# Jiraiya812/Fast-CU-Decision-HEVC

Hardware: AMD Instinct MI355X
Metric: CTUs/sec (RDO decision only) at 4K all-intra (higher is better)
Workload: dtype int32+f64

## Files before the change

fast-cu-decision-hevc_amd/csrc/fcu_engine.h:

```cpp
#pragma once
#include <stdint.h>
#include <string.h>
#include <type_traits>
#include "../../include/fcu.h"

#ifdef FCU_EMU
#include <math.h>
#include <stdio.h>
#include <stdlib.h>
#define FCU_DEV static inline
#define FCU_MEMBER inline
#define FCU_NOINLINE
#define FCU_INLINE
#define FCU_TABLE static const
static int g_emu_phase = 0, g_emu_in_phase = 0, g_emu_lane = 0, g_emu_relax = 0;
#define FCU_EMU_RELAX(on) (g_emu_relax = (on))
static inline int fcu_emu_phase_begin() { g_emu_phase++; g_emu_in_phase = 1; g_emu_lane = 0; return 0; }
static inline int fcu_emu_phase_next(int lane) { if (lane + 1 >= 64) g_emu_in_phase = 0; g_emu_lane = lane + 1; return lane + 1; }
template <class T> static inline T fcu_emu_uni(T v, int site, int line)
{
  enum { SITES = 2048, K = 32, B = 16 };
  struct Seen { int phase, first, cur, idx, n; unsigned char vals[K][B]; };
  static Seen seen[SITES];
  if (g_emu_in_phase && !g_emu_relax && sizeof(T) <= B && site < SITES) {
// ... 106 lines not shown
#define FCU_TIC(v) do { } while (0)
#define FCU_TOC(E_, v, idx) do { } while (0)
#define FCU_COUNT(E_, idx, n) do { } while (0)
#endif
#ifndef FCU_QTOC
#define FCU_QTIC(v) do { } while (0)
#define FCU_QTOC(E_, v, idx) do { } while (0)
#endif
#ifndef FCU_ITOC
#define FCU_ITOC(E_, v, idx) do { } while (0)
#endif
#ifndef FCU_MTOC
#define FCU_MTOC(E_, v, idx) do { } while (0)
#endif
#ifndef FCU_STOC
#define FCU_STOC(E_, v, idx) do { } while (0)
#define FCU_SPATH(E_, path) do { } while (0)
#define FCU_S7_COEFF(E_, v, comp) do { } while (0)
#endif

#include "fcu_tables.h"

struct HotTables { uint32_t bin[256]; uint16_t scan[3][16]; uint8_t scan_cg8[3][4]; uint8_t ctx_ind_map4x4[16]; uint8_t group_idx[32];
                   uint64_t scan4_nib[3], map4_nib; uint32_t cnt_bits[4]; };
#ifdef FCU_EMU
static HotTables g_hot;
#else
__shared__ HotTables g_hot;
#endif

#if defined(FCU_PROFILE_RQT) && !defined(FCU_EMU)
#define FCU_RTIC(v) long long v = clock64()
#define FCU_RTOC(P_, v, idx) do { if (!SER && threadIdx.x == 0) { ((Chain *)((char *)&(P_) - __builtin_offsetof(Chain, p)))->prof[idx] += (unsigned long long)(clock64() - v); v = clock64(); } } while (0)
#elif defined(FCU_PROFILE_RDOQ) && !defined(FCU_EMU)
#define FCU_RTIC(v) long long v = clock64()
#define FCU_RTOC(P_, v, idx) do { if ((FCU_PROFILE_RDOQ + 0) == 2 ? (!SER && threadIdx.x == 0) : SER) { ((Chain *)((char *)&(P_) - __builtin_offsetof(Chain, p)))->prof[idx] += (unsigned long long)(clock64() - v); v = clock64(); } } while (0)
#else
#define FCU_RTIC(v) do { } while (0)
#define FCU_RTOC(P_, v, idx) do { } while (0)
#endif
namespace fcu {

enum { CTU = 64, MAXDEPTH = 3, NPART = 256, LOG2_MAXTU = 5, LOG2_MINTU = 2, TU_MAXDEPTH_INTRA = 3 };
enum { SIZE_2Nx2N = 0, SIZE_2NxN = 1, SIZE_Nx2N = 2, SIZE_NxN = 3, SIZE_2NxnU = 4, SIZE_2NxnD = 5, SIZE_nLx2N = 6, SIZE_nRx2N = 7, SIZE_NONE = 8, MODE_INTER = 0, MODE_INTRA = 1, MODE_NONE = 2 };
enum { SLICE_I = 0, SLICE_P = 1 };
enum { PLANAR = 0, DC = 1, HOR = 10, VER = 26, DM_CHROMA = 36 };
enum { CTX_SPLIT = 0, CTX_PARTSIZE = 3, CTX_INTRA_LUMA = 4, CTX_CHROMA_PRED = 5, CTX_CBF_LUMA = 6, CTX_CBF_CHROMA = 11,
// ... 87 lines not shown
  Cabac c64_state[5][4]; uint32_t c64_distk[5][4];
  Yuv16 resi_cu, resi_best, qt_resi[4];
  Yuv tmp_pred;
  uint8_t me_pred[9][CTU * CTU];
  int16_t me_h[3][72 * 64];
  int par_ps[4];
  int memo_valid[4][MEMO_K], memo_next[4], memo_zero[4][MEMO_K];
  int16_t memo_mv[4][MEMO_K][NPART][2]; int8_t memo_ref[4][MEMO_K][NPART];
  uint8_t memo_tr_idx[4][MEMO_K][NPART], memo_cbf[4][MEMO_K][3][NPART], memo_tskip[4][MEMO_K][3][NPART];
  alignas(16) int16_t memo_coef[MEMO_K * MEMO_POOL], memo_resi[MEMO_K * MEMO_POOL];
};

struct Env { Chain *C; Scratch *G; int cur_ctu, slice_start; int16_t tx0, ty0, tx1, ty1; };
FCU_DEV int in_tile(const Env E, int cx, int cy) { return cx >= E.tx0 && cx < E.tx1 && cy >= E.ty0 && cy < E.ty1; }
struct TU { int log2, tr_depth, part, nparts, x, y, off_y, cw, cwo, cx, cy, c_tr_depth, c_code_all, off_c, cu_depth, plast; };

struct Shared {
  Cabac cab[1 + (MAXDEPTH + 1) + MAXLC + 1];
  uint8_t ref5[5][68]; int dc5[5]; uint32_t cm_dist[5];
  union {
    int16_t lane_abs[MAXLC][32];
    RdoqRec rq_rec[16];
    int32_t rq_grp[16][MAXVC];
    struct {
      int32_t colsum[128];
      union {
        struct { uint8_t ref[264], reff[264]; };
        uint8_t ref5b[5][68];
      };
    };
  };
  union {
    int16_t rq_lv[16];
    uint32_t sad[36];
  };
  int dc;
  int ref_tag;
  int best_idx[4], reco_best_idx[4];
  union {
    struct { int rd_mode[12]; int n_rd; int preds[3]; int n_mpm; };
    int uni[8];
  };
  union {
    struct {
      uint8_t vc_slot[MAXVC];
      int vc_abs[MAXVC], vc_lsp[MAXVC], vc_last[MAXVC]; uint32_t vc_dist[MAXVC]; uint32_t vc_bits[MAXVC]; double vc_cost[MAXVC];
// ... 158 lines not shown
  int offset;
  if (log2 == 2) offset = g_hot.ctx_ind_map4x4[4 * py + px];
  else {
    int cnt; const int xs = px & 3, ys = py & 3;
    if (pattern == 0) { int t = xs + ys; cnt = (t >= 3) ? 0 : ((t >= 1) ? 1 : 2); }
    else if (pattern == 1) cnt = (ys >= 2) ? 0 : ((ys >= 1) ? 1 : 2);
    else if (pattern == 2) cnt = (xs >= 2) ? 0 : ((xs >= 1) ? 1 : 2);
    else cnt = 2;
    offset = ((((px >> 2) + (py >> 2)) > 0) ? (ch ? 0 : 3) : 0) + cnt;
  }
  return first + offset;
}
FCU_DEV int coef_remain_bins(uint32_t symbol, uint32_t rparam)
{
  int code = (int)symbol;
  if (code < (3 << rparam)) return (int)(((uint32_t)code >> rparam) + 1) + (int)rparam;
  uint32_t length = rparam;
  code -= 3 << rparam;
  while (code >= (1 << length)) code -= 1 << (length++);
  return (int)(3 + length + 1 - rparam) + (int)length;
}
#ifdef FCU_EMU
enum { WALK_RDOQ_CALLS, WALK_RDOQ_TOP_IS_GROUP0, WALK_RDOQ_AHEAD_GROUPS, WALK_RDOQ_ONLY_GROUP0, WALK_RDOQ_ONLY_LAST_GROUP, WALK_RDOQ_ALL_ZERO,
       WALK_BITS_CALLS, WALK_BITS_ONE_EMPTY_RUN_BETWEEN, WALK_BITS_SECOND_ROUND, WALK_N };
extern "C" { __attribute__((weak)) unsigned long long fcu_emu_walk_cnt[WALK_N]; }
static const int32_t *g_emu_lscan_lo = nullptr, *g_emu_lscan_hi = nullptr;
#define FCU_WALK_COUNT(i, n) (fcu_emu_walk_cnt[i] += (unsigned long long)(n))
#define FCU_CHECK_LSCAN(p) FCU_CHECK((const int32_t *)(p) >= g_emu_lscan_lo && (const int32_t *)(p) < g_emu_lscan_hi)
#else
#define FCU_WALK_COUNT(i, n) do { } while (0)
#define FCU_CHECK_LSCAN(p) do { } while (0)
#endif
template <int SER>
FCU_DEV FCU_INLINE void code_coeff_body(int c, const int16_t *coef, int st, int last, int log2, int comp, int scanType, int tsFlag, const Params &P_, int16_t *absCoeff)
{
  if (SER) { c = FCU_UNI(c); coef = FCU_UNI(coef); last = FCU_UNI(last); scanType = FCU_UNI(scanType); tsFlag = FCU_UNI(tsFlag); absCoeff = FCU_UNI(absCoeff); }
  const Params &P = *FCU_UNI(&P_);
  st = FCU_UNI(st); log2 = FCU_UNI(log2); comp = FCU_UNI(comp);
  FCU_IN_LDS(absCoeff);
  const FCU_HBM int16_t *coefg = (const FCU_HBM int16_t *)coef;
  const int ch = comp ? 1 : 0, N = 1 << log2; int n2 = N * N;
  if (last < 0 && st == 1 && n2 >= 64) {
    int q = (n2 >> 6) - 1;
    for (; q >= 0; q--) {
      uint32_t w[32];
      __builtin_memcpy(w, __builtin_assume_aligned((const void *)(coef + q * 64), 16), 128);
      uint32_t any = 0;
#pragma unroll
      for (int k = 0; k < 32; k++) any |= w[k];
      if (any) break;
    }
    if (q < 0) return;
    n2 = (q + 1) * 64;
  }
// ... 209 lines not shown
          for (int n = (lastCG == 1 ? last : 15); n >= 0; --n) {
            if (lv[n] != 0) {
              if (du[n] > 0) { curCost = -du[n]; curChange = 1; }
              else if (n == first && iabs(lv[n]) == 1) curCost = 0x7fffffff;
              else { curCost = du[n]; curChange = -1; }
            } else if (n < first) {
              const unsigned thisSign = srcg[(sub + n) * st] >= 0 ? 0 : 1;
              if (thisSign != signbit) curCost = 0x7fffffff; else { curCost = -du[n]; curChange = 1; }
            } else { curCost = -du[n]; curChange = 1; }
            if (curCost < minCostInc) { minCostInc = curCost; finalChange = curChange; minPos = n; }
          }
          if (lv[minPos] == 32767 || lv[minPos] == -32768) finalChange = -1;
          const int nv = srcg[(sub + minPos) * st] >= 0 ? lv[minPos] + finalChange : lv[minPos] - finalChange;
          dstg[(sub + minPos) * st] = (int16_t)nv;
        }
      }
      if (lastCG == 1) lastCG = 0;
    }
  }
  for (int sp = cgTop * 16 + 15; sp >= 0; sp--) if (dstg[sp * st]) { o.last = sp; break; }
  return o;
}

template <class CB>
FCU_DEV FCU_INLINE int rdoq_last_pos(CB cb, const FCU_HBM int16_t *dstg, const FCU_HBM RdoqRec *recg, const FCU_HBM double *cgg,
                                     int st, int log2, int ch, int scanType, int cbfCtx, const uint16_t *scan, const uint8_t *scanCG,
                                     uint64_t cgflag, int cgLastScanPos, int lastScanPos, double baseCost, double blockUncodedCost, double lambda)
{
  const int N = 1 << log2;
  double bestCost; int bestLastIdxP1 = 0;
  bestCost = blockUncodedCost + lambda * (double)cb(cbfCtx, 0);
  baseCost += lambda * (double)cb(cbfCtx, 1);
  const int lcc = log2 - 2, loff = ch ? 0 : (lcc * 3 + ((lcc + 1) >> 2)), lsh = ch ? lcc : ((lcc + 3) >> 2);
  const int lbx = CTX_LASTX + (ch ? 15 : 0) + loff, lby = CTX_LASTY + (ch ? 15 : 0) + loff, lgmax = g_hot.group_idx[N - 1];
  int foundLast = 0;
  for (int cgScanPos = cgLastScanPos; cgScanPos >= 0; cgScanPos--) {
    const int cgBlk = scanCG[cgScanPos];
    baseCost -= cgg[cgScanPos * st];
    if ((cgflag >> cgBlk) & 1) {
      const int top = (cgScanPos * 16 + 15 > lastScanPos) ? lastScanPos - cgScanPos * 16 : 15;
      int aLv = dstg[(cgScanPos * 16 + top) * st]; double aCs = recg[(cgScanPos * 16 + top) * st].cs;
      for (int posInCG = top; posInCG >= 0; posInCG--) {
        const int scanPos = cgScanPos * 16 + posInCG;
        const int lv = aLv; const double curCs = aCs;
        if (posInCG > 0) { aLv = dstg[(scanPos - 1) * st]; aCs = recg[(scanPos - 1) * st].cs; }
        if (lv) {
          const int blk = scan[scanPos];
          const int py = blk >> log2, px = blk - (py << log2);
          const int ax = scanType == 2 ? py : px, ay = scanType == 2 ? px : py;
          const int gx = g_hot.group_idx[ax], gy = g_hot.group_idx[ay];
          int bxs = 0, bys = 0;
          for (int k = 0; k < gx; k++) bxs += cb(lbx + (k >> lsh), 1);
          if (gx < lgmax) bxs += cb(lbx + (gx >> lsh), 0);
          for (int k = 0; k < gy; k++) bys += cb(lby + (k >> lsh), 1);
          if (gy < lgmax) bys += cb(lby + (gy >> lsh), 0);
          double r = (double)(bxs + bys);
          if (gx > 3) r += 32768.0 * (double)((gx - 2) >> 1);
          if (gy > 3) r += 32768.0 * (double)((gy - 2) >> 1);
          const double costLast = lambda * r;
          const double totalCost = baseCost + costLast - curCs;
          if (totalCost < bestCost) { bestLastIdxP1 = scanPos + 1; bestCost = totalCost; }
          if (lv > 1) { foundLast = 1; break; }
          baseCost -= recg[scanPos * st].cc; baseCost += recg[scanPos * st].c0;
        } else baseCost -= curCs;
      }
      if (foundLast) break;
    }
  }
  return bestLastIdxP1;
}
FCU_DEV FCU_INLINE int rdoq_signs(const FCU_HBM int32_t *srcg, FCU_HBM int16_t *dstg, int st, int bestLastIdxP1, int lastScanPos)
{
  int absSum = 0;
  for (int sp0 = 0; sp0 < bestLastIdxP1; sp0 += 16) {
    int lv[16]; int32_t sv[16];
#pragma unroll
    for (int k = 0; k < 16; k++) { const int ok = sp0 + k < bestLastIdxP1; lv[k] = ok ? dstg[(sp0 + k) * st] : 0; sv[k] = ok ? srcg[(sp0 + k) * st] : 0; }
#pragma unroll
    for (int k = 0; k < 16; k++) if (sp0 + k < bestLastIdxP1) { absSum += lv[k]; dstg[(sp0 + k) * st] = (int16_t)((sv[k] < 0) ? -lv[k] : lv[k]); }
  }
  for (int sp = bestLastIdxP1; sp <= lastScanPos; sp++) dstg[sp * st] = 0;

  return absSum;
}
FCU_DEV FCU_INLINE void rdoq_sign_hiding(const Params &P, const FCU_HBM int32_t *srcg, FCU_HBM int16_t *dstg, const FCU_HBM RdoqRec *recg, int st, int ch, int bestLastIdxP1, int absSum)
{
  if (P.sign_hiding && absSum >= 2) {
    const long long rdFactor = P.rd_factor[ch];
    int lastCG = -1;
    for (int subSet = (bestLastIdxP1 - 1) >> 4; subSet >= 0; subSet--) {
      const int subPos = subSet << 4; int firstNZ = 16, lastNZ = -1, sum = 0, n;
      uint32_t nzMask = 0, negMask = 0;
      {
        int lv16[16];
#pragma unroll
        for (int k = 0; k < 16; k++) lv16[k] = dstg[(subPos + k) * st];
#pragma unroll
        for (int k = 0; k < 16; k++) { sum += lv16[k]; nzMask |= (uint32_t)(lv16[k] != 0) << k; negMask |= (uint32_t)(lv16[k] < 0) << k; }
      }
      if (nzMask) { lastNZ = 31 - __builtin_clz(nzMask); firstNZ = __builtin_ctz(nzMask); }
      if (lastNZ >= 0 && lastCG == -1) lastCG = 1;
      if (lastNZ - firstNZ >= 4) {
        const uint32_t signbit = (negMask >> firstNZ) & 1;
        if (signbit != (uint32_t)(sum & 1)) {
          long long minCostInc = 0x7fffffffffffffffLL, curCost = 0x7fffffffffffffffLL;
          int minPos = -1, finalChange = 0, curChange = 0;
          for (n = (lastCG == 1 ? lastNZ : 15); n >= 0; --n) {
            const int sp = n + subPos; const int lv = dstg[sp * st]; const RdoqRec q = recg[sp * st];
            if (lv != 0) {
              const long long costUp = rdFactor * (-q.du) + q.up;
              long long costDown = rdFactor * (q.du) + q.dn - ((iabs(lv) == 1) ? q.sd : 0);
              if (lastCG == 1 && lastNZ == n && iabs(lv) == 1) costDown -= (4 << 15);
              if (costUp < costDown) { curCost = costUp; curChange = 1; }
              else { curChange = -1; if (n == firstNZ && iabs(lv) == 1) curCost = 0x7fffffffffffffffLL; else curCost = costDown; }
            } else {
              curCost = rdFactor * (-(long long)(iabs(q.du))) + (1 << 15) + q.up + q.sd;
              curChange = 1;
              if (n < firstNZ) { const uint32_t thissign = srcg[sp * st] >= 0 ? 0 : 1; if (thissign != signbit) curCost = 0x7fffffffffffffffLL; }
            }
            if (curCost < minCostInc) { minCostInc = curCost; finalChange = curChange; minPos = sp; }
          }
          const int old = dstg[minPos * st];
          if (old == 32767 || old == -32768) finalChange = -1;
          const int nv = srcg[minPos * st] >= 0 ? old + finalChange : old - finalChange;
          dstg[minPos * st] = (int16_t)nv;
        }
      }
      if (lastCG == 1) lastCG = 0;
    }
  }
}
template <int SER, class CB>
FCU_DEV FCU_INLINE RdoqOut rdoq_finish(CB cb, const Params &P, const FCU_HBM int32_t *srcg, FCU_HBM int16_t *dstg, FCU_HBM RdoqRec *recg, FCU_HBM double *cgg,
                                       int st, int log2, int ch, int scanType, int cbfCtx, const uint16_t *scan, const uint8_t *scanCG,
                                       uint64_t cgflag, int cgLastScanPos, int lastScanPos, double baseCost, double blockUncodedCost, double lambda)
{
  FCU_RTIC(rt_);
  const int bestLastIdxP1 = rdoq_last_pos(cb, dstg, recg, cgg, st, log2, ch, scanType, cbfCtx, scan, scanCG, cgflag, cgLastScanPos, lastScanPos, baseCost, blockUncodedCost, lambda);
  FCU_RTOC(P, rt_, 13);
  const int absSum = rdoq_signs(srcg, dstg, st, bestLastIdxP1, lastScanPos);
  FCU_RTOC(P, rt_, 14);
  rdoq_sign_hiding(P, srcg, dstg, recg, st, ch, bestLastIdxP1, absSum);
  FCU_RTOC(P, rt_, 15);
  int last = bestLastIdxP1 - 1;
  while (last >= 0 && dstg[last * st] == 0) last--;
  RdoqOut o = { absSum, last };
  return o;
}


template <int SER, int EST>
FCU_DEV FCU_NOINLINE RdoqOut rdoq(int c, const int32_t *src, int16_t *dst, int st, int topNZ, int log2, int comp, int scanType, int cbfCtx, const Params &P_, RdoqRec *rec, double *costCGSig, int slot = 0)
{
  const Params &P = *FCU_UNI(&P_);
  st = FCU_UNI(st); log2 = FCU_UNI(log2); comp = FCU_UNI(comp); cbfCtx = FCU_UNI(cbfCtx);
  if (SER) { c = FCU_UNI(c); src = FCU_UNI(src); dst = FCU_UNI(dst); topNZ = FCU_UNI(topNZ); scanType = FCU_UNI(scanType); rec = FCU_UNI(rec); costCGSig = FCU_UNI(costCGSig); }
  FCU_RTIC(rt_);
  if (topNZ < 0) { FCU_WALK_COUNT(WALK_RDOQ_ALL_ZERO, !SER); RdoqOut z = { 0, -1 }; return z; }
  const FCU_HBM int32_t *srcg = (const FCU_HBM int32_t *)src; FCU_HBM int16_t *dstg = (FCU_HBM int16_t *)dst;
  FCU_HBM RdoqRec *recg = (FCU_HBM RdoqRec *)rec; FCU_HBM double *cgg = (FCU_HBM double *)costCGSig;
  auto cb = [&](int ctx, int bin) -> int { return EST ? (int)FCU_EST[ctx * 2 + bin] : ctx_bits(c, ctx, bin); };
  const int ch = comp ? 1 : 0, N = 1 << log2, n2 = N * N;
  const int qp = comp ? P.qp_c : P.qp;
  const int qbits = rdoq_qbits(log2, qp);
  const double lambda = P.rdoq_lambda[comp];
  const double errScale = P.err_scale[ch][log2 - 2];
  const uint16_t *scan = log2 == 2 ? &g_hot.scan[scanType][0] : k_scan + k_scan_off[scanType * 4 + log2 - 2];
  const uint8_t *scanCG = log2 <= 3 ? g_hot.scan_cg8[log2 == 2 ? 0 : scanType] : k_scan_cg + k_scan_cg_off[scanType * 4 + log2 - 2];
  const int wg = N >> 2, firstSig = first_sig_ctx(log2, scanType, ch);
  const int sigOff = CTX_SIG + (ch ? 28 : 0), cgBase = CTX_SIGCG + (ch ? 2 : 0);
  uint64_t cgflag = 0;
  int cgLastScanPos = -1; uint32_t ctxSet = 0; int c1 = 1, c2 = 0;
  double baseCost = 0, blockUncodedCost = 0;
  int lastScanPos = -1; uint32_t c1Idx = 0, c2Idx = 0, goRice = 0;
  int absSum = 0;

  const uint64_t scan4 = g_hot.scan4_nib[scanType], map4 = g_hot.map4_nib;
  int g10 = 0, g10Ctx = -1;
  const int cgTop = topNZ >> 4;
  for (int cg = (n2 >> 4) - 1; cg > cgTop; cg--) {
    int32_t v[16];
#pragma unroll
    for (int k = 0; k < 16; k++) v[k] = srcg[(cg * 16 + k) * st];
#pragma unroll
    for (int k = 15; k >= 0; k--) { const double err = (double)iabs(v[k]); blockUncodedCost += err * err * errScale; }
  }
  baseCost = blockUncodedCost;
  FCU_RTOC(P, rt_, 11);
  constexpr bool GRP = !SER;
  int32_t ahead = 0, nxt[16];
  if (GRP) {
// ... 101 lines not shown
        rdCodedLevelandDist += cc - cs;
        rdUncodedDist += c0;
        if (posInCG != 0) nnzBeforePos0++;
      }
    }
    if (lastScanPos >= 0 && cgScanPos > 0) {
      ctxSet = (uint32_t)((ch ? 4 : 0) + ((!ch && (cgScanPos - 1) > 0) ? 2 : 0) + (c1 == 0));
      c1 = 1; c2 = 0; c1Idx = 0; c2Idx = 0; goRice = 0;
    }
    if (cgLastScanPos >= 0) {
      if (cgScanPos) {
        if (((cgflag >> cgBlk) & 1) == 0) {
          const int ctxSig = cgBase + sig_cg_ctx(cgflag, cgx, cgy, wg);
          baseCost += lambda * (double)cb(ctxSig, 0) - rdSigCost;
          cgg[cgScanPos * st] = lambda * (double)cb(ctxSig, 0);
        } else if (cgScanPos < cgLastScanPos) {
          if (nnzBeforePos0 == 0) { baseCost -= rdSigCost0; rdSigCost -= rdSigCost0; }
          double costZeroCG = baseCost;
          const int ctxSig = cgBase + sig_cg_ctx(cgflag, cgx, cgy, wg);
          baseCost += lambda * (double)cb(ctxSig, 1);
          costZeroCG += lambda * (double)cb(ctxSig, 0);
          cgg[cgScanPos * st] = lambda * (double)cb(ctxSig, 1);
          costZeroCG += rdUncodedDist; costZeroCG -= rdCodedLevelandDist; costZeroCG -= rdSigCost;
          if (costZeroCG < baseCost) {
            cgflag &= ~(1ull << cgBlk); baseCost = costZeroCG;
            cgg[cgScanPos * st] = lambda * (double)cb(ctxSig, 0);
            for (int posInCG = 15; posInCG >= 0; posInCG--) {
              const int scanPos = cgScanPos * 16 + posInCG;
              if (SER) { if (g_S.rq_lv[posInCG]) { g_S.rq_lv[posInCG] = 0; g_S.rq_rec[posInCG].cc = g_S.rq_rec[posInCG].c0; g_S.rq_rec[posInCG].cs = 0; } }
              else if (dstg[scanPos * st]) { dstg[scanPos * st] = 0; recg[scanPos * st].cc = recg[scanPos * st].c0; recg[scanPos * st].cs = 0; }
            }
          }
        }
      } else cgflag |= 1ull << cgBlk;
    }
    if (SER) {
#pragma unroll
      for (int k = 0; k < 16; k++) { recg[(cgScanPos * 16 + k) * st] = g_S.rq_rec[k]; dstg[(cgScanPos * 16 + k) * st] = g_S.rq_lv[k]; }
    }
  }
  FCU_RTOC(P, rt_, 12);
  if (lastScanPos < 0) { RdoqOut z = { 0, -1 }; return z; }
#ifdef FCU_EMU
  FCU_WALK_COUNT(WALK_RDOQ_ONLY_GROUP0, GRP && lastScanPos < 16);
  if (GRP && n2 > 16 && lastScanPos >= n2 - 16) {
    int other = 0;
    for (int sp = 0; sp < n2 - 16; sp++) other |= dstg[sp * st];
    FCU_WALK_COUNT(WALK_RDOQ_ONLY_LAST_GROUP, !other);
  }
#endif
  return rdoq_finish<SER>(cb, P, srcg, dstg, recg, cgg, st, log2, ch, scanType, cbfCtx, scan, scanCG, cgflag, cgLastScanPos, lastScanPos, baseCost, blockUncodedCost, lambda);
}

#ifdef FCU_EMU
template <class T> struct LaneVar {
  T v[64];
  LaneVar() { for (int i = 0; i < 64; i++) v[i] = T(); }
  void set(int lane, T x) { v[lane] = x; }
  T own(int lane) const { return v[lane]; }
  T get(int k) const { return v[k]; }
  void put(int k, T x) { v[k] = x; }
};
FCU_DEV uint32_t lane_mask16(const LaneVar<int> &f) { uint32_t m = 0; for (int k = 0; k < 16; k++) m |= (uint32_t)(f.v[k] != 0) << k; return m; }
#else
#if defined(__HIP_DEVICE_COMPILE__)
#define FCU_READLANE(v, k) __builtin_amdgcn_readlane((v), (k))
#define FCU_WRITELANE(val_, k_, old_) (((int)threadIdx.x == (k_)) ? (val_) : (old_))
#define FCU_BALLOT(p) __builtin_amdgcn_ballot_w64(p)
#else
#define FCU_READLANE(v, k) (v)
#define FCU_WRITELANE(val_, k_, old_) (val_)
#define FCU_BALLOT(p) ((unsigned long long)(p))
#endif
template <class T> struct LaneVar;
// ... 14 lines not shown
  { union { double d; int i[2]; } u, w; u.d = r; w.d = x; u.i[0] = FCU_WRITELANE(w.i[0], k, u.i[0]); u.i[1] = FCU_WRITELANE(w.i[1], k, u.i[1]); r = u.d; }
};
__device__ inline uint32_t lane_mask16(const LaneVar<int> &f) { return (uint32_t)FCU_BALLOT(f.r != 0) & 0xffffu; }
#endif

#ifndef FCU_WAVE_RDOQ_MIN_LOG2
#define FCU_WAVE_RDOQ_MIN_LOG2 2
#endif
FCU_DEV FCU_NOINLINE void rdoq_wave(int c, const int32_t *src, int16_t *dst, int topNZ, int log2, int comp, int scanType, int cbfCtx, const Params &P_, RdoqRec *rec, double *costCGSig)
{
  const Params &P = *FCU_UNI(&P_);
  c = FCU_UNI(c); src = FCU_UNI(src); dst = FCU_UNI(dst); topNZ = FCU_UNI(topNZ); log2 = FCU_UNI(log2); comp = FCU_UNI(comp);
  scanType = FCU_UNI(scanType); cbfCtx = FCU_UNI(cbfCtx); rec = FCU_UNI(rec); costCGSig = FCU_UNI(costCGSig);
  if (topNZ < 0) { FCU_SERIAL { g_S.rw_abs = 0; g_S.rw_lsp = -1; } return; }
  const FCU_HBM int32_t *srcg = (const FCU_HBM int32_t *)src; FCU_HBM int16_t *dstg = (FCU_HBM int16_t *)dst;
  FCU_HBM RdoqRec *recg = (FCU_HBM RdoqRec *)rec; FCU_HBM double *cgg = (FCU_HBM double *)costCGSig;
  auto cb = [&](int ctx, int bin) -> int { return (int)FCU_EST[ctx * 2 + bin]; };
  const int ch = comp ? 1 : 0, N = 1 << log2, n2 = N * N;
  const int qp = comp ? P.qp_c : P.qp;
  const int qbits = rdoq_qbits(log2, qp);
  const double lambda = P.rdoq_lambda[comp];
  const double errScale = P.err_scale[ch][log2 - 2];
  const uint16_t *scan = log2 == 2 ? &g_hot.scan[scanType][0] : k_scan + k_scan_off[scanType * 4 + log2 - 2];
  const uint8_t *scanCG = log2 <= 3 ? g_hot.scan_cg8[log2 == 2 ? 0 : scanType] : k_scan_cg + k_scan_cg_off[scanType * 4 + log2 - 2];
  const int wg = N >> 2, firstSig = first_sig_ctx(log2, scanType, ch);
  const int sigOff = CTX_SIG + (ch ? 28 : 0), cgBase = CTX_SIGCG + (ch ? 2 : 0);
  const uint64_t scan4 = g_hot.scan4_nib[scanType], map4 = g_hot.map4_nib;
  const int cgTop = topNZ >> 4;
  uint64_t cgflag = 0;
  int cgLastScanPos = -1; uint32_t ctxSet = 0; int c1 = 1, c2 = 0;
  double baseCost = 0, blockUncodedCost = 0;
  int lastScanPos = -1; uint32_t c1Idx = 0, c2Idx = 0, goRice = 0;
  int g10 = 0, g10Ctx = -1;
  for (int cg = (n2 >> 4) - 1; cg > cgTop; cg -= 4) {
    LaneVar<double> t0;
    FCU_FOR_LANES { const int g = cg - (lane >> 4); if (g > cgTop) { const double err = (double)iabs(srcg[g * 16 + (lane & 15)]); t0.set(lane, err * err * errScale); } }
    for (int j = 0; j < 4 && cg - j > cgTop; j++)
      for (int k = 15; k >= 0; k--) blockUncodedCost += t0.get(j * 16 + k);
  }
  baseCost = blockUncodedCost;
  LaneVar<int> vCgBlk, vNext;
  LaneVar<double> vCgSig;
  FCU_FOR_LANES { if (lane <= cgTop) vCgBlk.set(lane, scanCG[lane]); if (lane < 16) vNext.set(lane, srcg[cgTop * 16 + lane]); }
  for (int cgScanPos = cgTop; cgScanPos >= 0; cgScanPos--) {
    const int cgBlk = vCgBlk.get(cgScanPos), cgy = cgBlk / wg, cgx = cgBlk - cgy * wg;
    const int sigBase = sigOff + firstSig + ((!ch && (cgx + cgy) > 0) ? 3 : 0);
    const uint32_t cntBits = g_hot.cnt_bits[pattern_sig_ctx(cgflag, cgx, cgy, wg)];
// ... 171 lines not shown
      }
      for (int posInCG = top; posInCG >= 0; posInCG--) {
        const int lv = wLv.get(posInCG); const double curCs = wCs.get(posInCG);
        if (lv) {
          const double totalCost = baseCost + wCl.get(posInCG) - curCs;
          if (totalCost < bestCost) { bestLastIdxP1 = cgScanPos * 16 + posInCG + 1; bestCost = totalCost; }
          if (lv > 1) { foundLast = 1; break; }
          baseCost -= wCc.get(posInCG); baseCost += wC0.get(posInCG);
        } else baseCost -= curCs;
      }
    }
  }
  FCU_SERIAL { g_S.rw_abs = 0; }
  FCU_FOR_LANES {
    uint32_t acc = 0;
    for (int sp = lane; sp <= lastScanPos; sp += 64) {
      if (sp < bestLastIdxP1) { const int lv = dstg[sp]; acc += (uint32_t)lv; dstg[sp] = (int16_t)((srcg[sp] < 0) ? -lv : lv); }
      else dstg[sp] = 0;
    }
    FCU_WAVE_ADD((uint32_t *)&g_S.rw_abs, acc);
  }
  FCU_SERIAL {
    const int absSum = g_S.rw_abs;
    rdoq_sign_hiding(P, srcg, dstg, recg, 1, ch, bestLastIdxP1, absSum);
    int last = bestLastIdxP1 - 1;
    while (last >= 0 && dstg[last] == 0) last--;
    g_S.rw_lsp = last;
  }
}

FCU_DEV int use_filtered_ref(int mode, int log2, int isLuma)
{
  if (!isLuma || mode == DC) return 0;
  const int d1 = iabs(mode - HOR), d2 = iabs(mode - VER);
  return (d1 < d2 ? d1 : d2) > k_filter_thr[log2 - 2];
}
FCU_DEV int pred_pixel(const uint8_t *ref, int log2, int mode, int isLuma, int dc, int x, int y)
{
  const int N = 1 << log2;
  const uint8_t *corner = ref + 2 * N;
  if (mode == PLANAR)
    return ((N - 1 - x) * corner[-1 - y] + (x + 1) * corner[1 + N] + (N - 1 - y) * corner[1 + x] + (y + 1) * corner[-1 - N] + N) >> (log2 + 1);
  if (mode == DC) {
    int v = dc;
    if (isLuma && N <= 16) {
      if (x == 0 && y == 0) v = (corner[1] + corner[-1] + 2 * dc + 2) >> 2;
      else if (y == 0) v = (corner[1 + x] + 3 * dc + 2) >> 2;
      else if (x == 0) v = (corner[-1 - y] + 3 * dc + 2) >> 2;
    }
// ... 1869 lines not shown
      if (!((depth < ctu->depth[part] && depth < MAXDEPTH) || boundary)) {
        encode_cu_syntax(E, c, ctu, part, depth);
        const int rx = cx + s, ry = cy + s;
        if (((rx % CTU) == 0 || rx == P.width) && ((ry % CTU) == 0 || ry == P.height) && !lastCtuOfSlice) cab_trm(c, 0);
        sp--; continue;
      }
      stChild[sp] = 0;
    }
    if (stChild[sp] >= 4) { sp--; continue; }
    {
      const int qn = (NPART >> (2 * depth)) >> 2, p = part + stChild[sp] * qn;
      stChild[sp]++;
      if (ctu->x + part_x(p) < P.width && ctu->y + part_y(p) < P.height) { sp++; stPart[sp] = p; stChild[sp] = -1; }
    }
  }
}

FCU_DEV void load_hot_tables()
{
  FCU_FOR_LANES {
    for (int i = lane; i < 256; i += 64) g_hot.bin[i] = k_bin[i];
    for (int i = lane; i < 3 * 16; i += 64) { const int t = i / 16, j = i % 16; g_hot.scan[t][j] = k_scan[k_scan_off[t * 4 + 0] + j]; }
    if (lane < 12) g_hot.scan_cg8[lane / 4][lane % 4] = k_scan_cg[k_scan_cg_off[(lane / 4) * 4 + 1] + lane % 4];
    if (lane < 16) g_hot.ctx_ind_map4x4[lane] = k_ctx_ind_map4x4[lane];
    if (lane < 32) g_hot.group_idx[lane] = k_group_idx[lane];
    if (lane < 3) { uint64_t v = 0; for (int j = 0; j < 16; j++) v |= (uint64_t)k_scan[k_scan_off[lane * 4 + 0] + j] << (4 * j); g_hot.scan4_nib[lane] = v; }
    if (lane == 3) { uint64_t v = 0; for (int j = 0; j < 16; j++) v |= (uint64_t)k_ctx_ind_map4x4[j] << (4 * j); g_hot.map4_nib = v; }
    if (lane >= 4 && lane < 8) {
      const int pattern = lane - 4; uint32_t v = 0;
      for (int j = 0; j < 16; j++) {
        const int xs = j & 3, ys = j >> 2; int cnt;
        if (pattern == 0) { const int t = xs + ys; cnt = (t >= 3) ? 0 : ((t >= 1) ? 1 : 2); }
        else if (pattern == 1) cnt = (ys >= 2) ? 0 : ((ys >= 1) ? 1 : 2);
        else if (pattern == 2) cnt = (xs >= 2) ? 0 : ((xs >= 1) ? 1 : 2);
        else cnt = 2;
        v |= (uint32_t)cnt << (2 * j);
      }
      g_hot.cnt_bits[pattern] = v;
    }
  }
}

template <bool WPP = false>
FCU_DEV FCU_NOINLINE void compress_ctu(Chain *C, Scratch *G, int pos)
{
  C = FCU_UNI(C); G = FCU_UNI(G); pos = FCU_UNI(pos);
  Env E; E.C = C; E.G = G;
#ifdef FCU_EMU
  g_emu_lscan_lo = G->p_lscan; g_emu_lscan_hi = G->p_lscan + POOL;
#endif
  FCU_TIC(t10_);
  const Params &P = C->p;
  const int tileW = FCU_UNI(C->tile_w), tileX0 = FCU_UNI(C->tile_x0), tileY0 = FCU_UNI(C->tile_y0);
  const int col = pos % tileW;
  const int ctuRsAddr = FCU_UNI((tileY0 + pos / tileW) * C->w_ctu + tileX0 + col);
  E.tx0 = (int16_t)tileX0; E.ty0 = (int16_t)tileY0; E.tx1 = (int16_t)(tileX0 + tileW); E.ty1 = (int16_t)(tileY0 + FCU_UNI(C->tile_h));
  const int sliceLen = P.slice_ctus > 0 ? P.slice_ctus : C->n_ctu;
  const int sliceStart = (ctuRsAddr / sliceLen) * sliceLen;
  int sliceEnd = sliceStart + sliceLen; if (sliceEnd > C->n_ctu) sliceEnd = C->n_ctu;
  E.cur_ctu = ctuRsAddr; E.slice_start = sliceStart;
  fcu_ctu_out *out = &C->out[ctuRsAddr];
  const int x = (ctuRsAddr % C->w_ctu) * CTU, y = (ctuRsAddr / C->w_ctu) * CTU;
  const bool unit_start = ctuRsAddr == sliceStart || pos == 0;
  const bool row_start = WPP && col == 0 && !unit_start;
  FCU_SERIAL { g_S.env = E; g_S.ref_tag = -1; if (unit_start || row_start) cab_init(slot_ptr(E, 0, CI_CURR_BEST), P.qp, P.slice_type, P.cabac_b_table); else cab_copy1(slot_ptr(E, 0, CI_CURR_BEST), &C->state); }
  if (row_start && tileW >= 2) {
    const uint8_t *src = C->wpp_sync_in;
    FCU_FOR_LANES { Cabac *d = slot_ptr(E, 0, CI_CURR_BEST); for (int i = lane; i < NCTX; i += 64) d->ctx[i] = src[i]; }
  }
  FCU_FOR_LANES {
    for (int i = lane; i < NPART; i += 64) {
      out->depth[i] = 0; out->width[i] = CTU; out->height[i] = CTU; out->skip[i] = 0; out->part_size[i] = SIZE_NONE; out->pred_mode[i] = MODE_NONE;
// ... 112 lines not shown
```

Baseline: 20210.

## Prefetch RDOQ tail data in half-groups and cache scan tables in LDS

The last-position search in RDOQ now walks the coefficients in blocks of eight. It loads each block's levels and cost records ahead of use and stages the cs values in shared memory per slot, so global loads overlap with the serial cost evaluation. Sign hiding now batch-loads its record fields per half-group and returns the last nonzero position, which removes the separate backward scan; a mask-based helper covers the case without sign hiding. The 16x16 and 32x32 CG scan tables are copied into the shared hot-table struct. The cost is extra shared memory and more registers, plus emulator-only bounds checks and counters.

```diff
diff --git a/fast-cu-decision-hevc_amd/csrc/fcu_engine.h b/fast-cu-decision-hevc_amd/csrc/fcu_engine.h
--- a/fast-cu-decision-hevc_amd/csrc/fcu_engine.h
+++ b/fast-cu-decision-hevc_amd/csrc/fcu_engine.h
@@ -152,7 +152,8 @@
 #include "fcu_tables.h"
 
 struct HotTables { uint32_t bin[256]; uint16_t scan[3][16]; uint8_t scan_cg8[3][4]; uint8_t ctx_ind_map4x4[16]; uint8_t group_idx[32];
-                   uint64_t scan4_nib[3], map4_nib; uint32_t cnt_bits[4]; };
+                   uint64_t scan4_nib[3], map4_nib; uint32_t cnt_bits[4];
+                   uint8_t scan_cg16[16], scan_cg32[64]; };
 #ifdef FCU_EMU
 static HotTables g_hot;
 #else
@@ -286,6 +287,7 @@
     int16_t lane_abs[MAXLC][32];
     RdoqRec rq_rec[16];
     int32_t rq_grp[16][MAXVC];
+    double rq_cs[8][MAXVC];
     struct {
       int32_t colsum[128];
       union {
@@ -490,14 +492,24 @@
 }
 #ifdef FCU_EMU
 enum { WALK_RDOQ_CALLS, WALK_RDOQ_TOP_IS_GROUP0, WALK_RDOQ_AHEAD_GROUPS, WALK_RDOQ_ONLY_GROUP0, WALK_RDOQ_ONLY_LAST_GROUP, WALK_RDOQ_ALL_ZERO,
-       WALK_BITS_CALLS, WALK_BITS_ONE_EMPTY_RUN_BETWEEN, WALK_BITS_SECOND_ROUND, WALK_N };
-extern "C" { __attribute__((weak)) unsigned long long fcu_emu_walk_cnt[WALK_N]; }
+       WALK_BITS_CALLS, WALK_BITS_ONE_EMPTY_RUN_BETWEEN, WALK_BITS_SECOND_ROUND, WALK_N,
+       TAIL_LAST_IN_GROUP0 = WALK_N, TAIL_LAST_AT_POS15, TAIL_LAST_AT_POS0, TAIL_SEARCH_ENDS_IN_FIRST_GROUP, TAIL_SEARCH_THREE_GROUPS,
+       TAIL_NOTHING_CODED, TAIL_HIDE_MINPOS_BELOW_FIRST, TAIL_HIDE_MINPOS_IS_LAST_ONE, TAIL_BIG_TU_DIAGONAL, TAIL_ZERO_OUT_TAKEN,
+       TAIL_ZERO_OUT_NOT_TAKEN, WALK_ALL };
+extern "C" { __attribute__((weak)) unsigned long long fcu_emu_walk_cnt[WALK_ALL]; __attribute__((weak)) int fcu_emu_walk_n[2] = { WALK_N, WALK_ALL }; }
 static const int32_t *g_emu_lscan_lo = nullptr, *g_emu_lscan_hi = nullptr;
+static const void *g_emu_qscan_lo = nullptr, *g_emu_qscan_hi = nullptr, *g_emu_rec_lo = nullptr, *g_emu_rec_hi = nullptr, *g_emu_cg_lo = nullptr, *g_emu_cg_hi = nullptr;
 #define FCU_WALK_COUNT(i, n) (fcu_emu_walk_cnt[i] += (unsigned long long)(n))
 #define FCU_CHECK_LSCAN(p) FCU_CHECK((const int32_t *)(p) >= g_emu_lscan_lo && (const int32_t *)(p) < g_emu_lscan_hi)
+#define FCU_CHECK_QSCAN(p) FCU_CHECK((const void *)(p) >= g_emu_qscan_lo && (const void *)((p) + 1) <= g_emu_qscan_hi)
+#define FCU_CHECK_REC(p) FCU_CHECK((const void *)(p) >= g_emu_rec_lo && (const void *)((p) + 1) <= g_emu_rec_hi)
+#define FCU_CHECK_CG(p) FCU_CHECK((const void *)(p) >= g_emu_cg_lo && (const void *)((p) + 1) <= g_emu_cg_hi)
 #else
 #define FCU_WALK_COUNT(i, n) do { } while (0)
 #define FCU_CHECK_LSCAN(p) do { } while (0)
+#define FCU_CHECK_QSCAN(p) do { } while (0)
+#define FCU_CHECK_REC(p) do { } while (0)
+#define FCU_CHECK_CG(p) do { } while (0)
 #endif
 template <int SER>
 FCU_DEV FCU_INLINE void code_coeff_body(int c, const int16_t *coef, int st, int last, int log2, int comp, int scanType, int tsFlag, const Params &P_, int16_t *absCoeff)
@@ -753,10 +765,16 @@
   return o;
 }
 
+FCU_DEV FCU_INLINE const uint8_t *hot_scan_cg(int log2, int scanType)
+{
+  FCU_CHECK(log2 <= 3 || scanType == 0);
+  return log2 <= 3 ? g_hot.scan_cg8[log2 == 2 ? 0 : scanType] : (log2 == 4 ? g_hot.scan_cg16 : g_hot.scan_cg32);
+}
+
 template <class CB>
 FCU_DEV FCU_INLINE int rdoq_last_pos(CB cb, const FCU_HBM int16_t *dstg, const FCU_HBM RdoqRec *recg, const FCU_HBM double *cgg,
                                      int st, int log2, int ch, int scanType, int cbfCtx, const uint16_t *scan, const uint8_t *scanCG,
-                                     uint64_t cgflag, int cgLastScanPos, int lastScanPos, double baseCost, double blockUncodedCost, double lambda)
+                                     uint64_t cgflag, int cgLastScanPos, int lastScanPos, double baseCost, double blockUncodedCost, double lambda, int slot)
 {
   const int N = 1 << log2;
   double bestCost; int bestLastIdxP1 = 0;
@@ -764,40 +782,64 @@
   baseCost += lambda * (double)cb(cbfCtx, 1);
   const int lcc = log2 - 2, loff = ch ? 0 : (lcc * 3 + ((lcc + 1) >> 2)), lsh = ch ? lcc : ((lcc + 3) >> 2);
   const int lbx = CTX_LASTX + (ch ? 15 : 0) + loff, lby = CTX_LASTY + (ch ? 15 : 0) + loff, lgmax = g_hot.group_idx[N - 1];
-  int foundLast = 0;
-  for (int cgScanPos = cgLastScanPos; cgScanPos >= 0; cgScanPos--) {
-    const int cgBlk = scanCG[cgScanPos];
-    baseCost -= cgg[cgScanPos * st];
-    if ((cgflag >> cgBlk) & 1) {
-      const int top = (cgScanPos * 16 + 15 > lastScanPos) ? lastScanPos - cgScanPos * 16 : 15;
-      int aLv = dstg[(cgScanPos * 16 + top) * st]; double aCs = recg[(cgScanPos * 16 + top) * st].cs;
-      for (int posInCG = top; posInCG >= 0; posInCG--) {
-        const int scanPos = cgScanPos * 16 + posInCG;
-        const int lv = aLv; const double curCs = aCs;
-        if (posInCG > 0) { aLv = dstg[(scanPos - 1) * st]; aCs = recg[(scanPos - 1) * st].cs; }
-        if (lv) {
-          const int blk = scan[scanPos];
-          const int py = blk >> log2, px = blk - (py << log2);
-          const int ax = scanType == 2 ? py : px, ay = scanType == 2 ? px : py;
-          const int gx = g_hot.group_idx[ax], gy = g_hot.group_idx[ay];
-          int bxs = 0, bys = 0;
-          for (int k = 0; k < gx; k++) bxs += cb(lbx + (k >> lsh), 1);
-          if (gx < lgmax) bxs += cb(lbx + (gx >> lsh), 0);
-          for (int k = 0; k < gy; k++) bys += cb(lby + (k >> lsh), 1);
-          if (gy < lgmax) bys += cb(lby + (gy >> lsh), 0);
-          double r = (double)(bxs + bys);
-          if (gx > 3) r += 32768.0 * (double)((gx - 2) >> 1);
-          if (gy > 3) r += 32768.0 * (double)((gy - 2) >> 1);
-          const double costLast = lambda * r;
-          const double totalCost = baseCost + costLast - curCs;
-          if (totalCost < bestCost) { bestLastIdxP1 = scanPos + 1; bestCost = totalCost; }
-          if (lv > 1) { foundLast = 1; break; }
-          baseCost -= recg[scanPos * st].cc; baseCost += recg[scanPos * st].c0;
-        } else baseCost -= curCs;
-      }
-      if (foundLast) break;
-    }
-  }
+  int foundLast = 0, flagged = 0, walked = 0;
+  const int hTop = lastScanPos >> 3;
+  FCU_CHECK(slot >= 0 && slot < MAXVC && cgLastScanPos == (lastScanPos >> 4));
+  FCU_WALK_COUNT(TAIL_LAST_IN_GROUP0, lastScanPos < 16); FCU_WALK_COUNT(TAIL_LAST_AT_POS15, (lastScanPos & 15) == 15); FCU_WALK_COUNT(TAIL_LAST_AT_POS0, (lastScanPos & 15) == 0);
+  int nLv[8]; double nCs[8];
+#pragma unroll
+  for (int k = 0; k < 8; k++) { const int i = (hTop * 8 + k) * st; FCU_CHECK_QSCAN(&dstg[i]); FCU_CHECK_REC(&recg[i]); nLv[k] = dstg[i]; nCs[k] = recg[i].cs; }
+  FCU_CHECK_CG(&cgg[cgLastScanPos * st]);
+  double nCg = cgg[cgLastScanPos * st];
+  for (int h = hTop; h >= 0; h--) {
+    const int cgScanPos = h >> 1;
+    uint32_t nz = 0, gt1 = 0;
+#pragma unroll
+    for (int k = 0; k < 8; k++) { g_S.rq_cs[k][slot] = nCs[k]; nz |= (uint32_t)(nLv[k] != 0) << k; gt1 |= (uint32_t)(nLv[k] > 1) << k; }
+    const int first = (h & 1) || h == hTop;
+    const double curCg = nCg;
+    if (first) {
+      const int below = cgScanPos > 0 ? cgScanPos - 1 : 0;
+      FCU_CHECK_CG(&cgg[below * st]); nCg = cgg[below * st];
+    }
+    if (h > 0) {
+#pragma unroll
+      for (int k = 0; k < 8; k++) { const int i = ((h - 1) * 8 + k) * st; FCU_CHECK_QSCAN(&dstg[i]); FCU_CHECK_REC(&recg[i]); nLv[k] = dstg[i]; nCs[k] = recg[i].cs; }
+    }
+    if (first) {
+      baseCost -= curCg;
+      flagged = (int)((cgflag >> scanCG[cgScanPos]) & 1);
+      walked += flagged;
+    }
+    if (!flagged) continue;
+    const int top = h == hTop ? (lastScanPos & 7) : 7;
+    for (int p = top; p >= 0; p--) {
+      const int scanPos = h * 8 + p;
+      const double curCs = g_S.rq_cs[p][slot];
+      if ((nz >> p) & 1) {
+        const double curCc = recg[scanPos * st].cc, curC0 = recg[scanPos * st].c0;
+        const int blk = scan[scanPos];
+        const int py = blk >> log2, px = blk - (py << log2);
+        const int ax = scanType == 2 ? py : px, ay = scanType == 2 ? px : py;
+        const int gx = g_hot.group_idx[ax], gy = g_hot.group_idx[ay];
+        int bxs = 0, bys = 0;
+        for (int k = 0; k < gx; k++) bxs += cb(lbx + (k >> lsh), 1);
+        if (gx < lgmax) bxs += cb(lbx + (gx >> lsh), 0);
+        for (int k = 0; k < gy; k++) bys += cb(lby + (k >> lsh), 1);
+        if (gy < lgmax) bys += cb(lby + (gy >> lsh), 0);
+        double r = (double)(bxs + bys);
+        if (gx > 3) r += 32768.0 * (double)((gx - 2) >> 1);
+        if (gy > 3) r += 32768.0 * (double)((gy - 2) >> 1);
+        const double costLast = lambda * r;
+        const double totalCost = baseCost + costLast - curCs;
+        if (totalCost < bestCost) { bestLastIdxP1 = scanPos + 1; bestCost = totalCost; }
+        if ((gt1 >> p) & 1) { foundLast = 1; break; }
+        baseCost -= curCc; baseCost += curC0;
+      } else baseCost -= curCs;
+    }
+    if (foundLast) break;
+  }
+  FCU_WALK_COUNT(TAIL_SEARCH_ENDS_IN_FIRST_GROUP, foundLast && walked == 1); FCU_WALK_COUNT(TAIL_SEARCH_THREE_GROUPS, walked - foundLast >= 3);
   return bestLastIdxP1;
 }
 FCU_DEV FCU_INLINE int rdoq_signs(const FCU_HBM int32_t *srcg, FCU_HBM int16_t *dstg, int st, int bestLastIdxP1, int lastScanPos)
@@ -814,67 +856,94 @@
 
   return absSum;
 }
-FCU_DEV FCU_INLINE void rdoq_sign_hiding(const Params &P, const FCU_HBM int32_t *srcg, FCU_HBM int16_t *dstg, const FCU_HBM RdoqRec *recg, int st, int ch, int bestLastIdxP1, int absSum)
-{
-  if (P.sign_hiding && absSum >= 2) {
-    const long long rdFactor = P.rd_factor[ch];
-    int lastCG = -1;
-    for (int subSet = (bestLastIdxP1 - 1) >> 4; subSet >= 0; subSet--) {
-      const int subPos = subSet << 4; int firstNZ = 16, lastNZ = -1, sum = 0, n;
-      uint32_t nzMask = 0, negMask = 0;
-      {
-        int lv16[16];
-#pragma unroll
-        for (int k = 0; k < 16; k++) lv16[k] = dstg[(subPos + k) * st];
-#pragma unroll
-        for (int k = 0; k < 16; k++) { sum += lv16[k]; nzMask |= (uint32_t)(lv16[k] != 0) << k; negMask |= (uint32_t)(lv16[k] < 0) << k; }
-      }
-      if (nzMask) { lastNZ = 31 - __builtin_clz(nzMask); firstNZ = __builtin_ctz(nzMask); }
-      if (lastNZ >= 0 && lastCG == -1) lastCG = 1;
-      if (lastNZ - firstNZ >= 4) {
-        const uint32_t signbit = (negMask >> firstNZ) & 1;
-        if (signbit != (uint32_t)(sum & 1)) {
-          long long minCostInc = 0x7fffffffffffffffLL, curCost = 0x7fffffffffffffffLL;
-          int minPos = -1, finalChange = 0, curChange = 0;
-          for (n = (lastCG == 1 ? lastNZ : 15); n >= 0; --n) {
-            const int sp = n + subPos; const int lv = dstg[sp * st]; const RdoqRec q = recg[sp * st];
+FCU_DEV FCU_INLINE int rdoq_last_level(const FCU_HBM int16_t *dstg, int st, int last)
+{
+  for (int cg = last >> 4; cg >= 0; cg--) {
+    uint32_t nz = 0;
+#pragma unroll
+    for (int k = 0; k < 16; k++) { FCU_CHECK_QSCAN(&dstg[(cg * 16 + k) * st]); nz |= (uint32_t)(dstg[(cg * 16 + k) * st] != 0) << k; }
+    if (cg == (last >> 4)) nz &= (2u << (last & 15)) - 1;
+    if (nz) return cg * 16 + 31 - __builtin_clz(nz);
+  }
+  return -1;
+}
+FCU_DEV FCU_INLINE int rdoq_sign_hiding(const Params &P, const FCU_HBM int32_t *srcg, FCU_HBM int16_t *dstg, const FCU_HBM RdoqRec *recg, int st, int ch, int bestLastIdxP1, int absSum)
+{
+  if (!(P.sign_hiding && absSum >= 2)) return -2;
+  const long long rdFactor = P.rd_factor[ch];
+  int lastCG = -1, last = -1;
+  for (int subSet = (bestLastIdxP1 - 1) >> 4; subSet >= 0; subSet--) {
+    const int subPos = subSet << 4; int firstNZ = 16, lastNZ = -1, sum = 0;
+    uint32_t nzMask = 0, negMask = 0;
+    int lv16[16];
+#pragma unroll
+    for (int k = 0; k < 16; k++) { FCU_CHECK_QSCAN(&dstg[(subPos + k) * st]); lv16[k] = dstg[(subPos + k) * st]; }
+#pragma unroll
+    for (int k = 0; k < 16; k++) { sum += lv16[k]; nzMask |= (uint32_t)(lv16[k] != 0) << k; negMask |= (uint32_t)(lv16[k] < 0) << k; }
+    if (nzMask) { lastNZ = 31 - __builtin_clz(nzMask); firstNZ = __builtin_ctz(nzMask); }
+    if (lastNZ >= 0 && lastCG == -1) lastCG = 1;
+    if (lastNZ - firstNZ >= 4) {
+      const uint32_t signbit = (negMask >> firstNZ) & 1;
+      if (signbit != (uint32_t)(sum & 1)) {
+        long long minCostInc = 0x7fffffffffffffffLL, curCost = 0x7fffffffffffffffLL;
+        int minPos = -1, finalChange = 0, curChange = 0, minLv = 0, minNeg = 0;
+        const int nTop = lastCG == 1 ? lastNZ : 15;
+#pragma unroll
+        for (int half = 1; half >= 0; half--) {
+          int32_t du[8], up[8], dn[8], sd[8], sv[8];
+#pragma unroll
+          for (int k = 0; k < 8; k++) {
+            const int i = (subPos + half * 8 + k) * st;
+            FCU_CHECK_REC(&recg[i]); FCU_CHECK_LSCAN(&srcg[i]);
+            du[k] = recg[i].du; up[k] = recg[i].up; dn[k] = recg[i].dn; sd[k] = recg[i].sd; sv[k] = srcg[i];
+          }
+#pragma unroll
+          for (int k = 7; k >= 0; k--) {
+            const int n = half * 8 + k;
+            if (n > nTop) continue;
+            const int lv = lv16[n];
             if (lv != 0) {
-              const long long costUp = rdFactor * (-q.du) + q.up;
-              long long costDown = rdFactor * (q.du) + q.dn - ((iabs(lv) == 1) ? q.sd : 0);
+              const long long costUp = rdFactor * (-du[k]) + up[k];
+              long long costDown = rdFactor * (du[k]) + dn[k] - ((iabs(lv) == 1) ? sd[k] : 0);
               if (lastCG == 1 && lastNZ == n && iabs(lv) == 1) costDown -= (4 << 15);
               if (costUp < costDown) { curCost = costUp; curChange = 1; }
               else { curChange = -1; if (n == firstNZ && iabs(lv) == 1) curCost = 0x7fffffffffffffffLL; else curCost = costDown; }
             } else {
-              curCost = rdFactor * (-(long long)(iabs(q.du))) + (1 << 15) + q.up + q.sd;
+              curCost = rdFactor * (-(long long)(iabs(du[k]))) + (1 << 15) + up[k] + sd[k];
               curChange = 1;
-              if (n < firstNZ) { const uint32_t thissign = srcg[sp * st] >= 0 ? 0 : 1; if (thissign != signbit) curCost = 0x7fffffffffffffffLL; }
+              if (n < firstNZ) { const uint32_t thissign = sv[k] >= 0 ? 0 : 1; if (thissign != signbit) curCost = 0x7fffffffffffffffLL; }
             }
-            if (curCost < minCostInc) { minCostInc = curCost; finalChange = curChange; minPos = sp; }
+            if (curCost < minCostInc) { minCostInc = curCost; finalChange = curChange; minPos = n; minLv = lv; minNeg = sv[k] < 0; }
           }
-          const int old = dstg[minPos * st];
-          if (old == 32767 || old == -32768) finalChange = -1;
-          const int nv = srcg[minPos * st] >= 0 ? old + finalChange : old - finalChange;
-          dstg[minPos * st] = (int16_t)nv;
-        }
-      }
-      if (lastCG == 1) lastCG = 0;
-    }
-  }
+        }
+        FCU_CHECK(minPos >= 0);
+        FCU_WALK_COUNT(TAIL_HIDE_MINPOS_BELOW_FIRST, minPos < firstNZ); FCU_WALK_COUNT(TAIL_HIDE_MINPOS_IS_LAST_ONE, minPos == lastNZ && iabs(minLv) == 1);
+        const int old = minLv;
+        if (old == 32767 || old == -32768) finalChange = -1;
+        const int nv = !minNeg ? old + finalChange : old - finalChange;
+        dstg[(subPos + minPos) * st] = (int16_t)nv;
+        nzMask = (nzMask & ~(1u << minPos)) | ((uint32_t)((int16_t)nv != 0) << minPos);
+      }
+    }
+    if (last < 0 && nzMask) last = subPos + 31 - __builtin_clz(nzMask);
+    if (lastCG == 1) lastCG = 0;
+  }
+  return last;
 }
 template <int SER, class CB>
 FCU_DEV FCU_INLINE RdoqOut rdoq_finish(CB cb, const Params &P, const FCU_HBM int32_t *srcg, FCU_HBM int16_t *dstg, FCU_HBM RdoqRec *recg, FCU_HBM double *cgg,
                                        int st, int log2, int ch, int scanType, int cbfCtx, const uint16_t *scan, const uint8_t *scanCG,
-                                       uint64_t cgflag, int cgLastScanPos, int lastScanPos, double baseCost, double blockUncodedCost, double lambda)
+                                       uint64_t cgflag, int cgLastScanPos, int lastScanPos, double baseCost, double blockUncodedCost, double lambda, int slot)
 {
   FCU_RTIC(rt_);
-  const int bestLastIdxP1 = rdoq_last_pos(cb, dstg, recg, cgg, st, log2, ch, scanType, cbfCtx, scan, scanCG, cgflag, cgLastScanPos, lastScanPos, baseCost, blockUncodedCost, lambda);
+  const int bestLastIdxP1 = rdoq_last_pos(cb, dstg, recg, cgg, st, log2, ch, scanType, cbfCtx, scan, scanCG, cgflag, cgLastScanPos, lastScanPos, baseCost, blockUncodedCost, lambda, slot);
   FCU_RTOC(P, rt_, 13);
   const int absSum = rdoq_signs(srcg, dstg, st, bestLastIdxP1, lastScanPos);
   FCU_RTOC(P, rt_, 14);
-  rdoq_sign_hiding(P, srcg, dstg, recg, st, ch, bestLastIdxP1, absSum);
+  int last = rdoq_sign_hiding(P, srcg, dstg, recg, st, ch, bestLastIdxP1, absSum);
+  if (last == -2) last = rdoq_last_level(dstg, st, bestLastIdxP1 - 1);
   FCU_RTOC(P, rt_, 15);
-  int last = bestLastIdxP1 - 1;
-  while (last >= 0 && dstg[last * st] == 0) last--;
+  FCU_WALK_COUNT(TAIL_NOTHING_CODED, bestLastIdxP1 == 0);
   RdoqOut o = { absSum, last };
   return o;
 }
@@ -897,7 +966,7 @@
   const double lambda = P.rdoq_lambda[comp];
   const double errScale = P.err_scale[ch][log2 - 2];
   const uint16_t *scan = log2 == 2 ? &g_hot.scan[scanType][0] : k_scan + k_scan_off[scanType * 4 + log2 - 2];
-  const uint8_t *scanCG = log2 <= 3 ? g_hot.scan_cg8[log2 == 2 ? 0 : scanType] : k_scan_cg + k_scan_cg_off[scanType * 4 + log2 - 2];
+  const uint8_t *scanCG = hot_scan_cg(log2, scanType);
   const int wg = N >> 2, firstSig = first_sig_ctx(log2, scanType, ch);
   const int sigOff = CTX_SIG + (ch ? 28 : 0), cgBase = CTX_SIGCG + (ch ? 2 : 0);
   uint64_t cgflag = 0;
@@ -1045,6 +1114,7 @@
           costZeroCG += lambda * (double)cb(ctxSig, 0);
           cgg[cgScanPos * st] = lambda * (double)cb(ctxSig, 1);
           costZeroCG += rdUncodedDist; costZeroCG -= rdCodedLevelandDist; costZeroCG -= rdSigCost;
+          FCU_WALK_COUNT(costZeroCG < baseCost ? TAIL_ZERO_OUT_TAKEN : TAIL_ZERO_OUT_NOT_TAKEN, !SER);
           if (costZeroCG < baseCost) {
             cgflag &= ~(1ull << cgBlk); baseCost = costZeroCG;
             cgg[cgScanPos * st] = lambda * (double)cb(ctxSig, 0);
@@ -1065,14 +1135,15 @@
   FCU_RTOC(P, rt_, 12);
   if (lastScanPos < 0) { RdoqOut z = { 0, -1 }; return z; }
 #ifdef FCU_EMU
-  FCU_WALK_COUNT(WALK_RDOQ_ONLY_GROUP0, GRP && lastScanPos < 16);
+  FCU_WALK_COUNT(WALK_RDOQ_ONLY_GROUP0, GRP && lastScanPos < 16); FCU_WALK_COUNT(TAIL_BIG_TU_DIAGONAL, log2 >= 4);
+  if (GRP) for (int sp = lastScanPos + 1; sp < cgTop * 16 + 16; sp++) __builtin_memset((void *)&recg[sp * st], 0xff, sizeof(RdoqRec));
   if (GRP && n2 > 16 && lastScanPos >= n2 - 16) {
     int other = 0;
     for (int sp = 0; sp < n2 - 16; sp++) other |= dstg[sp * st];
     FCU_WALK_COUNT(WALK_RDOQ_ONLY_LAST_GROUP, !other);
   }
 #endif
-  return rdoq_finish<SER>(cb, P, srcg, dstg, recg, cgg, st, log2, ch, scanType, cbfCtx, scan, scanCG, cgflag, cgLastScanPos, lastScanPos, baseCost, blockUncodedCost, lambda);
+  return rdoq_finish<SER>(cb, P, srcg, dstg, recg, cgg, st, log2, ch, scanType, cbfCtx, scan, scanCG, cgflag, cgLastScanPos, lastScanPos, baseCost, blockUncodedCost, lambda, slot);
 }
 
 #ifdef FCU_EMU
@@ -1133,7 +1204,7 @@
   const double lambda = P.rdoq_lambda[comp];
   const double errScale = P.err_scale[ch][log2 - 2];
   const uint16_t *scan = log2 == 2 ? &g_hot.scan[scanType][0] : k_scan + k_scan_off[scanType * 4 + log2 - 2];
-  const uint8_t *scanCG = log2 <= 3 ? g_hot.scan_cg8[log2 == 2 ? 0 : scanType] : k_scan_cg + k_scan_cg_off[scanType * 4 + log2 - 2];
+  const uint8_t *scanCG = hot_scan_cg(log2, scanType);
   const int wg = N >> 2, firstSig = first_sig_ctx(log2, scanType, ch);
   const int sigOff = CTX_SIG + (ch ? 28 : 0), cgBase = CTX_SIGCG + (ch ? 2 : 0);
   const uint64_t scan4 = g_hot.scan4_nib[scanType], map4 = g_hot.map4_nib;
@@ -1351,9 +1422,8 @@
   }
   FCU_SERIAL {
     const int absSum = g_S.rw_abs;
-    rdoq_sign_hiding(P, srcg, dstg, recg, 1, ch, bestLastIdxP1, absSum);
-    int last = bestLastIdxP1 - 1;
-    while (last >= 0 && dstg[last] == 0) last--;
+    int last = rdoq_sign_hiding(P, srcg, dstg, recg, 1, ch, bestLastIdxP1, absSum);
+    if (last == -2) last = rdoq_last_level(dstg, 1, bestLastIdxP1 - 1);
     g_S.rw_lsp = last;
   }
 }
@@ -3269,6 +3339,8 @@
     for (int i = lane; i < 256; i += 64) g_hot.bin[i] = k_bin[i];
     for (int i = lane; i < 3 * 16; i += 64) { const int t = i / 16, j = i % 16; g_hot.scan[t][j] = k_scan[k_scan_off[t * 4 + 0] + j]; }
     if (lane < 12) g_hot.scan_cg8[lane / 4][lane % 4] = k_scan_cg[k_scan_cg_off[(lane / 4) * 4 + 1] + lane % 4];
+    if (lane < 16) g_hot.scan_cg16[lane] = k_scan_cg[k_scan_cg_off[2] + lane];
+    g_hot.scan_cg32[lane] = k_scan_cg[k_scan_cg_off[3] + lane];
     if (lane < 16) g_hot.ctx_ind_map4x4[lane] = k_ctx_ind_map4x4[lane];
     if (lane < 32) g_hot.group_idx[lane] = k_group_idx[lane];
     if (lane < 3) { uint64_t v = 0; for (int j = 0; j < 16; j++) v |= (uint64_t)k_scan[k_scan_off[lane * 4 + 0] + j] << (4 * j); g_hot.scan4_nib[lane] = v; }
@@ -3295,6 +3367,7 @@
   Env E; E.C = C; E.G = G;
 #ifdef FCU_EMU
   g_emu_lscan_lo = G->p_lscan; g_emu_lscan_hi = G->p_lscan + POOL;
+  g_emu_qscan_lo = G->p_qscan; g_emu_qscan_hi = G->p_qscan + POOL; g_emu_rec_lo = G->r_rec; g_emu_rec_hi = G->r_rec + POOL; g_emu_cg_lo = G->r_cg; g_emu_cg_hi = G->r_cg + MAXVC * 64;
 #endif
   FCU_TIC(t10_);
   const Params &P = C->p;
```

Measured after the change: 21380 (median of 6 runs). 1.06x the previous value.
